# neofytr/LLMTokenizer

Measured on AMD Instinct MI355X. Metric: corpus MB/s per merge iter (train), 1 GiB synthetic corpus, higher is better.
Workload: dtype u32

## Files before the change

### llmtokenizer_amd/csrc/batch.hip

```cpp
#pragma once
#include "engine_common.h"

namespace bpeamd {

static_assert(TOPK == 64, "a wave holds a list, one entry per lane");
static_assert(BRB == 2 * (1024 / 64), "the select's 16 waves merge two partial lists each");
#ifndef BPE_SU
#define BPE_SU 1
#endif
#ifndef BPE_FORM_PRINT
#define BPE_FORM_PRINT 0
#endif
#ifndef BPE_RU
#define BPE_RU 4
#endif
#ifndef BPE_AU
#define BPE_AU 1
#endif
constexpr uint32_t AU = BPE_AU;
constexpr uint32_t SU = BPE_SU;
#ifndef BPE_RUN_THREAD_PAIRS
#define BPE_RUN_THREAD_PAIRS 16
#endif
constexpr uint32_t RUN_THREAD_PAIRS = BPE_RUN_THREAD_PAIRS, RUN_Q = 256;
// ... 691 lines not shown
        const unsigned long long pcut = sh && ovm < k ? bank_shfl(pre, ovm - 1) : 0ull;
        unsigned long long sumlen = 0;
#pragma unroll
        for (uint32_t b = 0; b < NBK; b++) {
            const uint32_t q = 64 * b + lane;
            slot_k[b] = slot[b];
            if (sh && q >= ovm) len[b] = slot_k[b] = 0;
            if (sh && ovm < k && q >= ovm) pre[b] = pcut;
            sumlen += q < k ? len[b] : 0u;
        }
        const unsigned long long stage_end = bank_shfl(pre, k - 1);
        sumlen = wave_sum(sumlen);
        uint32_t wk[NBK];
        unsigned long long sumw = 0, big = 0;
#pragma unroll
        for (uint32_t b = 0; b < NBK; b++) {
            const uint32_t q = 64 * b + lane;
            wk[b] = q < k && mode[b] != 0 && E->scan_occd ? min(len[b], fm_c[q] + len[b] / E->scan_occd) : len[b];
            sumw += q < k ? wk[b] : 0u;
        }
        sumw = wave_sum(sumw);
#pragma unroll
        for (uint32_t b = 0; b < NBK; b++) {
            const uint32_t q = 64 * b + lane;
            nb[b] = q < k ? 1 + (uint32_t)(sumw ? (uint64_t)(BSB - k) * wk[b] / sumw : 0) : 0;
            bpre[b] = nb[b];
            if (q < k) big = max(big, ((unsigned long long)wk[b] << 8) | (255u - q));
        }
        bank_scan(bpre);
        for (int o = 32; o > 0; o >>= 1) big = max(big, (unsigned long long)__shfl_xor(big, o));
        const uint32_t used = bank_shfl(bpre, k - 1);
        const uint32_t bigm = 255u - (uint32_t)(big & 255u);
        const uint32_t extra = BSB - used;
#pragma unroll
        for (uint32_t b = 0; b < NBK; b++) {
            const uint32_t q = 64 * b + lane;
            if (q < k) {
                B->a[q] = fm_u[q];
                B->b[q] = fm_v[q];
                B->cnt[q] = fm_c[q];
                B->mode[q] = mode[b];
                B->off[q] = off[b];
                B->len[q] = len[b];
                B->sbase[q] = (uint32_t)(pre[b] - slot_k[b]);
                B->R[q] = 0;
                B->bound[q] = 0;
                B->blk0[q] = bpre[b] - nb[b] + (q > bigm ? extra : 0);
                B->tmask[q] = (uint8_t)fm_tm[q];
                B->tspan[q] = (uint32_t)min(fm_span[q], 0xFFFFFFFFull);
                ctl[q] = tl[b];
            }
        }
        const uint32_t nsk = k ? fm_nsk[k - 1] : 0u;
        if (lane == 0) {
            B->sbase[k] = (uint32_t)stage_end;
            B->blk0[k] = BSB;
            B->sumlen = (uint32_t)sumlen;
            B->over = ovm < k ? ovm : BK;
            B->tpend = tpend < k ? tpend : BK;
            Bg->nsk = nsk;
            Bg->gr_n = 0;
#pragma unroll
            for (uint32_t g = 0; g < GRUN; g++) {
                Bg->gr_tk[g] = 0;
                Bg->gr_endc[g] = 0xFFFFFFFFu;
                Bg->gr_ready[g] = 0;
            }
            B->ztot = 0;
            B->tbar = 0;
            B->tlog_n = 0;
            B->why[why_end]++;
            if (ties > 1) C->counters[2]++;
        }
        ts_mark(E, bi, BT_SEL_CAND, false);
    }
    if (tid < 64 && stop != STOP_NONE) k = 0;
    if (tid == 0) {
        if (B->sc_out && B->ap_out) {
            B->sc_ticks += B->sc_out - ~B->sc_in;
            B->ap_ticks += B->ap_out - ~B->ap_in;
            B->nspan++;
        }
        B->sc_in = B->sc_out = B->ap_in = B->ap_out = 0;
        B->rhold = stop != STOP_NONE ? retry : 0u;
        Bg->nstall = nst;
        if (stalled && !C->err) C->err = 10;
        B->skgate = (stop == STOP_NONE && !retry && skg ? skg - 1u : skg) | (ske << 16);
        if (applied) {
            B->zrate = (uint32_t)min(2ull * B->nzero / (md ? md : 1u) + 2ull, 1ull << 20);
            Bg->crate = (uint32_t)min((unsigned long long)E->crate_pct * Bg->ncre / (100ull * (md ? md : 1u)) + 16ull, 1ull << 20);
            C->merges_done = md;
            C->occ_top += (uint32_t)rs;
            C->n_live = n_live;
            C->D = D;
            C->counters[0] += jst;
            C->counters[4] += oldsum;
            C->relist_c0 += rescan + ocand;
            C->relist_o0 += oocc;
            C->counters[5] += rs;
            if (jst) {
                C->a = olda;
                C->b = oldb;
                C->z = oldz0 + jst - 1;
            }
            if (retry) {
                B->nretry++;
                B->ndrop += kpr - retry;
            } else {
                B->nbatch++;
                B->ndrop += kpr - jst;
                Bg->nskip += oldnsk;
            }
            B->retry = 0;
            B->applied = 0;
            B->dD = 0;
        }
// ... 316 lines not shown

template <bool SH>
__device__ inline uint32_t cover_of(const uint32_t *__restrict__ tok, const RoleTab &rt, const BHalo &H, uint32_t p,
                                    int64_t ps, int64_t n) {
    if (!(rt.get(p) >> 31)) return BK;
    const int64_t pps = v_left<SH>(tok, ps);
    const uint32_t pp = tok_at_b<SH>(tok, H, pps, n);
    const uint32_t mm = rt.member(pp, p);
    if (mm >= BK || pp != p) return mm;
    uint32_t L;
    if (SH && ps < 0) {
        L = H.hlr[mm];
    } else {
        L = 1;
        int64_t x = v_left<SH>(tok, ps);
        for (; x >= 0 && tok[x] == p; x = v_left<SH>(tok, x)) L++;
        if (SH && x < 0) L += H.hlr[mm];
    }
    return (L & 1) ? BK : mm;
}

template <bool SH>
__device__ inline uint32_t starts_of(const uint32_t *__restrict__ tok, const RoleTab &rt, const BHalo &H, uint32_t q,
                                     int64_t kq, int64_t n) {
    const uint32_t lq = rt.get(q) & 0x7FFFFFFFu;
    if (!lq) return BK;
    const int64_t kn = v_right(kq, lq, n);
    return rt.member(q, tok_at_b<SH>(tok, H, kn, n));
}

enum : uint32_t { GRF_LGO = 1, GRF_LEND = 2, GRF_IGO = 3, GRF_IEND = 4 };
__device__ void bscan_long_runs(const Eng *__restrict__ E, Bat *__restrict__ B, const uint32_t *__restrict__ tok,
                                const RoleTab &rt, const BHalo &H, int64_t n, uint32_t z0, uint32_t sgen) {
    const uint32_t lane = threadIdx.x & 63;
    const uint32_t ng = uni(min(aload(&B->gr_n), GRUN));
    const uint64_t stride = gr_stride(E->n0), maxch = stride - 1;
    auto flag_of = [&](uint32_t st) { return (sgen << 3) | st; };
    for (uint32_t gi = 0; gi < ng; gi++) {
        uint32_t ok = 1;
        if (lane == 0) {
            const unsigned long long t0 = wall_clock64();
            while (__hip_atomic_load(&B->gr_ready[gi], __ATOMIC_ACQUIRE, __HIP_MEMORY_SCOPE_AGENT) != sgen) {
                if (wall_clock64() - t0 > E->gr_wait) {
                    ok = 0;
                    B->ra_err = 11;
                    atomicAdd(&B->gr_tready, 1u);
                    break;
                }
                __builtin_amdgcn_s_sleep(1);
            }
        }
        if (!uni((uint32_t)__shfl((int)ok, 0))) return;
        const uint32_t mg = uni(aload(&B->gr_m[gi])), ag = uni(B->a[mg]), zg = z0 + mg;
        const int64_t c0 = uni(aload(&B->gr_c[gi])), lag = uni(E->tlen[ag]);
        uint32_t *occg = E->ids_out + B->sbase[mg];
        uint16_t *tagg = E->btag + B->sbase[mg];
        const uint32_t slice = B->sbase[mg + 1] - B->sbase[mg];
        uint32_t *flags = E->grflag + (uint64_t)gi * stride;
        auto pos = [&](int64_t l) -> int64_t { return c0 + l * lag; };
        auto tk = [&](int64_t l) -> uint32_t {
            const int64_t p = pos(l);
            return p < n ? tok[p] : HOLE;
        };
        for (;;) {
            uint32_t chl = 0, endl = 0;
            if (lane == 0) {
                chl = atomicAdd(&B->gr_tk[gi], 1u);
// ... 101 lines not shown
                    npairs++;
                    if (q != HOLE) {
                        if (q == ag) nint_dr++;
                        else vadd_g(E, mg, V_DR, q, 1u);
                        if (rq == zg) nint_ir++;
                        else vadd_g(E, mg, V_IR, rq, 1u);
                    }
                }
              }
            }
            nint_dr = wave_sum(nint_dr);
            nint_ir = wave_sum(nint_ir);
            npairs = wave_sum(npairs);
            if (lane == 0) {
                vadd_g(E, mg, V_DR, ag, nint_dr);
                vadd_g(E, mg, V_IR, zg, nint_ir);
                if (npairs) atomicAdd(&B->bound[mg], npairs);
                atomicAdd(&B->nchunks, 1ull);
            }
#pragma unroll
            for (uint32_t bb = 0; bb < NBK; bb++) {
                unsigned long long tm = tadj.w[bb];
                for (int o = 32; o > 0; o >>= 1) tm |= __shfl_xor(tm, o);
                if (lane == 0 && tm) atomicOr(&B->adj[mg][bb], tm);
            }
        }
    }
}

template <bool SH>
__global__ __launch_bounds__(SCAN_T) void k_bscan(const Eng *__restrict__ E, const Ctl *__restrict__ C) {
    if (C->stop) return;
    Bat *B = E->bat;
    const uint32_t bi = bat_idx(E);
    ts_mark(E, bi, BT_SCAN_IN, true);
    if (threadIdx.x == 0) atomicMax(&B->sc_in, ~wall_clock64());
    __shared__ uint32_t s[4][DENSE];
    __shared__ uint32_t list[SCAN_T * SU * FR];
    __shared__ uint16_t ltag[SCAN_T * SU * FR];
    __shared__ uint32_t lcount, gbase, list_n, covc, sm, sk, sz0, bRs;
    __shared__ uint32_t lr_n, lr_brk, lr_pos[RUN_Q];
    __shared__ unsigned long long badj[NBK];
    __shared__ uint32_t gcnt[2];
    __shared__ uint32_t sa[BK], sb[BK];
    __shared__ RoleTab rt;
    __shared__ BHalo H;
    __shared__ uint32_t wmx[2][16];
    const uint32_t tid = threadIdx.x;
    const uint32_t sgen = ((uint32_t)(B->nbatch + B->nretry) & 0x0FFFFFFFu) + 1u;
    if (tid == 0) {
        sm = BK;
        covc = lcount = bRs = 0;
        lr_n = 0;
#pragma unroll
        for (uint32_t b = 0; b < NBK; b++) badj[b] = 0;
        gcnt[0] = gcnt[1] = 0;
        sk = B->k;
        sz0 = B->z0;
    }
    for (uint32_t q = tid; q < RH; q += SCAN_T) {
        rt.id[q] = HOLE;
        rt.fl[q] = 0;
    }
    for (uint32_t q = tid; q < RP; q += SCAN_T) rt.pk[q] = 0;
    uint32_t mla = 0;
    if (tid < BK) {
        const uint32_t lo = B->blk0[tid], hi = B->blk0[tid + 1];
        const uint32_t ma = B->a[tid];
        sa[tid] = ma;
        sb[tid] = B->b[tid];
        mla = E->tlen[ma];
        if (blockIdx.x >= lo && blockIdx.x < hi && tid < B->k) sm = tid;
    }
    __syncthreads();
    const uint32_t k = sk, m = sm, z0 = sz0;
    if (m >= k) {
        if (tid == 0) atomicMax(&B->sc_out, wall_clock64());
        return;
    }
    MK tadj = mk_zero();
    if (tid < k) {
        rt.put(sa[tid], sb[tid], mla, tid);
        if (SH) {
            Halo h;
            shard_halo(E->erec, E->nshards, E->shard, sa[tid], &h);
            H.hlr[tid] = h.hlrun;
            H.myi[tid] = h.myidx;
            if (tid == 0)
                for (int q = 0; q < 3; q++) {
                    H.HL[q] = h.HL[q];
                    H.HR[q] = h.HR[q];
                }
        }
    }
    const uint32_t a = sa[m], b = sb[m], z = z0 + m;
    const uint32_t la = E->tlen[a], lb = E->tlen[b];
    const uint32_t mode = B->mode[m], off = B->off[m], len = B->len[m];
    const uint32_t bid = blockIdx.x - B->blk0[m], nblk = B->blk0[m + 1] - B->blk0[m];
    const uint32_t sbase = B->sbase[m];
    uint32_t *occz = E->ids_out + sbase;
    uint16_t *tagz = E->btag + sbase;
    const uint32_t sslice = B->sbase[m + 1] - sbase;
#define STG(IDX, WHERE) if ((IDX) >= sslice) { B->ra_err = 12; } else
    uint32_t *Rm = &B->R[m];
    const int64_t n = (int64_t)E->n0;
    const uint32_t *__restrict__ tok = E->tok;
    const uint32_t want = mode == 2 ? a : b;
    const uint32_t lim = min(DENSE, z0 + k);
    for (uint32_t v = 0; v < 4; v++)
        for (uint32_t x = tid; x < lim; x += SCAN_T) s[v][x] = 0;
    __syncthreads();
    auto tok_at = [&](int64_t p) -> uint32_t { return tok_at_b<SH>(tok, H, p, n); };

    if (a != b) {
        static_assert(SU == 1 && BPE_WFLUSH, "the wave-driven candidate loop: one entry per lane per round");
        const uint32_t stride = nblk * SCAN_T;
        const uint32_t lane = tid & 63, wbase = (tid >> 6) * 64 * FR;
        uint32_t wcnt = 0, wocc = 0;
        uint32_t nent[SU];
        uint16_t ntg[SU];
        uint32_t eS = bid * SCAN_T + (tid & ~63u);
        auto load1 = [&](uint32_t s0, uint32_t &en, uint16_t &tg) {
            const uint32_t e = s0 + lane;
            en = 0;
            tg = 0xFFFFu;
            if (e < len) {
                en = mode == 0 ? E->plist[off + e] : E->occ[off + e];
                if (mode) tg = E->occnb[off + e];
            }
        };
        uint32_t pent = 0;
        uint16_t ptg = 0xFFFFu;
        auto advance = [&]() {
            eS += stride;
            if (SCAN_PD > 1) {
                nent[0] = pent;
                ntg[0] = ptg;
                if (eS + stride < len) load1(eS + stride, pent, ptg);
            } else if (eS < len) {
                load1(eS, nent[0], ntg[0]);
            }
        };
        auto flush = [&]() {
            __builtin_amdgcn_fence(__ATOMIC_RELEASE, "wavefront");
            __builtin_amdgcn_wave_barrier();
            uint32_t g = 0;
            if (lane == 0 && wcnt) g = atomicAdd(Rm, wcnt);
            g = __shfl(g, 0);
            for (uint32_t q = lane; q < wcnt; q += 64) {
                STG(g + q, "wflush") {
                occz[g + q] = list[wbase + q];
                tagz[g + q] = ltag[wbase + q];
                }
            }
// ... 281 lines not shown
                    }
                }
            }
            return fb < U;
        };
        if (nlr > RUN_BLOCK_Q) {
            for (uint32_t qi = wv; qi < nlr; qi += SCAN_T / 64) {
                int64_t c = lr_pos[qi];
                while (!segs(c, 0, std::integral_constant<uint32_t, 1>{}, [](uint32_t) { return 1u; }))
                    c += 64 * (int64_t)la;
            }
        } else {
            constexpr uint32_t NS = SCAN_T / 64 * RUN_BU;
            for (uint32_t qi = 0; qi < nlr; qi++) {
                int64_t c = lr_pos[qi];
                for (;;) {
                    if (tid == 0) lr_brk = NS;
                    __syncthreads();
                    segs(c, 64 * RUN_BU * wv, std::integral_constant<uint32_t, RUN_BU>{}, [&](uint32_t fb) {
                        if (lane == 0 && fb < RUN_BU) atomicMin(&lr_brk, wv * RUN_BU + fb);
                        __syncthreads();
                        const uint32_t gb = lr_brk, w0 = wv * RUN_BU;
                        return gb < w0 ? 0u : min(RUN_BU, gb - w0 + 1);
                    });
                    const bool done = lr_brk < NS;
                    __syncthreads();
                    if (done) break;
                    c += (int64_t)NS * 64 * la;
                }
            }
        }
    }
    __syncthreads();
    if (!SH && E->grflag) bscan_long_runs(E, B, tok, rt, H, n, z0, sgen);
    ts_mark(E, bi, BT_SCAN_CAND, false, true);
    if (tid < SKMAX && tid < B->nsk && ((B->sk_cm[tid][m >> 6] >> (m & 63)) & 1ull)) {
        const uint32_t xs = B->sk_a[tid], ys = B->sk_b[tid];
        uint32_t d = 0;
        if (xs == b && ys < lim) d += s[V_DR][ys];
        if (ys == a && xs < lim) d += s[V_DL][xs];
        if (d) atomicAdd(SH ? &E->xbat[BK + tid] : &B->sdec[tid], d);
    }
    const uint32_t Wx = xbat_vw(z0 + k);
    uint32_t *xm = SH ? E->xbat + XBH + (uint64_t)m * xbat_member_words(Wx) : nullptr;
    if (SH && blockIdx.x == 0 && tid == 0) {
        uint32_t xlm = BK;
        const int64_t F1 = C->F1, L1 = C->L1;
        const uint32_t over = B->over;
        if (F1 < n) {
            const uint32_t tf = tok[F1], tl1 = tok[L1];
            for (uint32_t mm = 0; mm < k; mm++)
                if (H.HL[0] == sa[mm] && tf == sb[mm] && (sa[mm] != sb[mm] || (H.hlr[mm] & 1))) {
                    xlm = mm;
                    break;
                }
            for (uint32_t mm = 0; mm < k && mm < over; mm++) {
                if (!(tl1 == sa[mm] && H.HR[0] == sb[mm] && (sa[mm] != sb[mm] || !(H.myi[mm] & 1)))) continue;
                uint32_t *xo = E->xbat + XBH + (uint64_t)mm * xbat_member_words(Wx);
                const uint32_t zz = z0 + mm;
                const int64_t ps = v_left<SH>(tok, L1);
                const uint32_t p = tok_at(ps);
                uint32_t lfin = p, bnd = 1;
                if (p != HOLE) {
                    const uint32_t cv = cover_of<SH>(tok, rt, H, p, ps, n);
                    if (cv < BK) {
                        lfin = z0 + cv;
                        bnd = 2;
                    } else {
                        xadd(E, xo, Wx, mm, V_DL, p);
                        xadd(E, xo, Wx, mm, V_IL, p);
                    }
                }
                const uint32_t q = H.HR[1];
                uint32_t rfin = q;
                if (q != HOLE) {
                    const uint32_t st = starts_of<SH>(tok, rt, H, q, n + 1, n);
                    if (st < BK) rfin = z0 + st;
                    xadd(E, xo, Wx, mm, V_DR, q);
                    xadd(E, xo, Wx, mm, V_IR, rfin);
                }
                (void)zz;
                const uint32_t g = atomicAdd(&B->R[mm], 1u);
                E->ids_out[B->sbase[mm] + g] = (uint32_t)L1;
                E->btag[B->sbase[mm] + g] = nb_tag(lfin, rfin);
                atomicAdd(&xo[0], 1u);
                atomicAdd(&xo[1], bnd);
                break;
            }
        }
        B->xl_m = xlm;
        if (over < k) atomicAdd(&E->xbat[over], 1u);
    }
    if (k > 1) {
#pragma unroll
        for (uint32_t bb = 0; bb < NBK; bb++) {
            unsigned long long t = tadj.w[bb];
            for (int o = 32; o > 0; o >>= 1) t |= __shfl_xor(t, o);
            if ((tid & 63) == 0 && t) atomicOr(&badj[bb], t);
        }
        __syncthreads();
        if (tid < NBK && badj[tid]) atomicOr(&B->adj[m][tid], badj[tid]);
    }
    uint32_t *rep = SH ? xm + 2 : E->bvecd + (uint64_t)(m * BREPL + bid % BREPL) * 4 * DENSE;
    const uint32_t vstride = SH ? Wx : DENSE;
    uint32_t mxl = 0, mxr = 0;
    for (uint32_t v = 0; v < 4; v++)
        for (uint32_t x = tid; x < lim; x += SCAN_T) {
            const uint32_t c = s[v][x];
            if (c) atomicAdd(&rep[v * vstride + x], c);
            if (v == V_DL) mxl = max(mxl, c);
            if (v == V_DR) mxr = max(mxr, c);
        }
    if (SH && tid == 0 && bRs) atomicAdd(&xm[0], bRs);
    if (k > 1) {
        for (int o = 32; o > 0; o >>= 1) {
            mxl = max(mxl, (uint32_t)__shfl_xor(mxl, o));
            mxr = max(mxr, (uint32_t)__shfl_xor(mxr, o));
        }
        if ((tid & 63) == 0) {
            wmx[0][tid >> 6] = mxl;
            wmx[1][tid >> 6] = mxr;
        }
        __syncthreads();
        if (tid == 0) {
            uint32_t l = 0, r = 0;
            for (uint32_t q = 0; q < SCAN_T / 64; q++) {
                l = max(l, wmx[0][q]);
                r = max(r, wmx[1][q]);
            }
            atomicAdd(SH ? &xm[1] : &B->bound[m], max(l + gcnt[V_DL] + covc, r + gcnt[V_DR]));
        }
    }
    ts_mark(E, bi, BT_SCAN_OUT, false, true);
    asm volatile("s_waitcnt vmcnt(0)" ::: "memory");
    __syncthreads();
    if (tid == 0) atomicMax(&B->sc_out, wall_clock64());
}
template __global__ void k_bscan<false>(const Eng *, const Ctl *);
template __global__ void k_bscan<true>(const Eng *, const Ctl *);

constexpr uint32_t XSP_SHIFT = 23;
static_assert(4 * BK < (1u << (32 - XSP_SHIFT)), "member-vector index fits above the id");
__global__ __launch_bounds__(256) void k_bpack(const Eng *__restrict__ E, const Ctl *__restrict__ C) {
    if (C->stop) return;
    const Bat *B = E->bat;
    __shared__ uint32_t pre[BK * 4 + 1];
    __shared__ uint32_t written;
    const uint32_t k = B->k, tid = threadIdx.x, nmv = 4 * k;
    if (tid < 64) {
        constexpr uint32_t LP = 4 * NBK;
        uint32_t c[LP], sum = 0;
#pragma unroll
        for (uint32_t j = 0; j < LP; j++) {
            c[j] = LP * tid + j < nmv ? E->bvnl[LP * tid + j] : 0u;
            sum += c[j];
        }
        uint32_t incl = sum;
        for (int o = 1; o < 64; o <<= 1) {
            const uint32_t y = __shfl_up(incl, o);
            if ((int)tid >= o) incl += y;
        }
        uint32_t r = incl - sum;
#pragma unroll
        for (uint32_t j = 0; j < LP; j++) {
            if (LP * tid + j <= nmv) pre[LP * tid + j] = r;
            r += c[j];
        }
    }
    __syncthreads();
// ... 637 lines not shown
```

### llmtokenizer_amd/csrc/engine.hip

```cpp
#include <hip/hip_runtime.h>
#include <fcntl.h>
#include <unistd.h>
#include <cerrno>

#include <algorithm>
#include <chrono>
#include <cstdio>
#include <cstdlib>
#include <cstring>
#include <string>
#include <thread>
#include <vector>
#include <unordered_map>

#include <rocprim/rocprim.hpp>

#include "../../include/bpe_gpu.h"
#include "kernels.hip"
#include "batch.hip"
#include "encode.hip"
#include "encode_win.hip"
#include "encode_docs.hip"
#include "split.hip"

// ... 189 lines not shown
            }
            return isnew == 1;
        };
        if (newt && is_new()) atomicAdd(&newt[t], 1u);
        const uint32_t bt = (uint32_t)(murmur_pair(u, v) & (C->Bfin[t] - 1));
        const uint32_t fc = E->sfirst[s];
        for (uint32_t q = 0; q < nq; q++) {
            if (qs[q].t != t) continue;
            if ((qs[q].flags & 1) && fc < qs[q].firstc) atomicAdd(&rho[q], 1u);
            if ((qs[q].flags & 2) && bt < qs[q].bucket && is_new()) atomicAdd(&nbl[q], 1u);
            if ((qs[q].flags & 4) && bt == qs[q].bucket) {
                const uint32_t p = atomicAdd(nmates, 1u);
                if (p < mcap) mates[p] = Mate{q, u, v, fc, is_new() ? 1u : 0u, 0};
            }
        }
    }
}

}

struct bpe_gpu_ctx {
    int dev = 0;
    hipStream_t st = nullptr;
    bool own_stream = true;
    uint32_t fast = 0;
    bool mlog_on = false;
    uint32_t sharded = 0, shard = 0, nshards = 1;
    uint64_t ntot = 0;
    uint32_t xfused = 0;
    uint32_t sbatch = 0;
    uint64_t stage_cap = 0;
    const P2P *xp2p = nullptr;
    unsigned long long xtimeout = 0;
    Eng h{};
    Eng *dE = nullptr;
    Ctl *dC = nullptr;
    Ctl *hC = nullptr;
    volatile uint32_t *hprobe = nullptr;
    hipEvent_t ev_probe[2] = {};
    uint64_t n0 = 0;
    bool loaded = false;
    bool ids_ready = false;
    uint64_t ids_len = 0;
    bool docs_ready = false;
    uint64_t docs_n = 0;
    uint64_t *d_idoff = nullptr;
    uint64_t docs_info[8] = {};
    bool split_ready = false;
    uint64_t split_n = 0;
    uint64_t *d_split = nullptr;
    size_t split_cap = 0;
    size_t merges_done = 0;
    std::vector<std::pair<void *, size_t>> train_allocs;
    std::vector<std::pair<void *, size_t>> pool;
    bool zdefer = false;
    std::vector<std::pair<void *, size_t>> zpend;
    uint32_t *d_tileoff = nullptr;
    uint32_t *d_enc_pairs = nullptr;
    hipGraphExec_t g_plain = nullptr, g_tracked = nullptr, g_encode = nullptr, g_batch = nullptr;
    bool hot_fallback = false;
    uint32_t relists = 0;
    std::vector<uint64_t> events;
    std::vector<hipGraphExec_t> retired;
    bpe_gpu_stats stats{};
    bool profile = false;
    hipEvent_t ev[2][ITERS_PER_GRAPH][2] = {};
// ... 243 lines not shown
                    (c->sharded ? c->sbatch != 0 : h.spec_on && (c->fast || n0 >= TRACK_LIMIT || HOT_TRACKED))
                ? 1
                : 0;
    h.relist_stale = 0;
    const bool will_batch = getenv_int("BPE_BATCH", 1) && h.hot;
    const int relist_env = getenv_int("BPE_RELIST", will_batch ? 1 : 0);
    if (!encode && !c->sharded && n0 >= (1ull << 24) && relist_env) {
        const char *t = getenv("BPE_RELIST_STALE");
        const uint64_t dflt = will_batch ? std::max<uint64_t>(n0 / 10, 1) : (32u << 20);
        h.relist_stale = (uint32_t)std::min<uint64_t>(t ? (uint64_t)std::max(1L, atol(t)) : dflt, 0xFFFFFFFFull);
    }
    h.hot_parts = SPEC_RB;
    h.hot_target = HOT_TARGET;
    if (const char *t = getenv("BPE_HOT_TARGET")) h.hot_target = std::max(1, std::min(atoi(t), (int)HOT_TARGET));
    h.hot_slot = h.hot_hist = h.hotp_tie = nullptr;
    h.hotp_best = h.hotp_key = h.hotp_v2 = h.hotp_k2 = nullptr;
    if (h.hot) {
        if ((r = dalloc(c, &h.hot_slot, HOT_CAP, false))) return r;
        if ((r = dalloc(c, &h.hot_hist, HOT_BINS))) return r;
        if ((r = dalloc(c, &h.hotp_best, SPEC_RB))) return r;
        if ((r = dalloc(c, &h.hotp_key, SPEC_RB))) return r;
        if ((r = dalloc(c, &h.hotp_v2, SPEC_RB))) return r;
        if ((r = dalloc(c, &h.hotp_k2, SPEC_RB))) return r;
        if ((r = dalloc(c, &h.hotp_tie, SPEC_RB))) return r;
    }
    h.batch = getenv_int("BPE_BATCH", 1) && h.hot && h.vcap <= BATCH_VCAP_MAX && (!c->sharded || c->sbatch) &&
                      (c->sharded || c->fast || n0 >= TRACK_LIMIT)
                  ? 1
                  : 0;
    h.skip_on = (uint32_t)(getenv_int("BPE_SKIP", 1) != 0);
    if (h.skip_on && getenv_int("BPE_SKIP_TEST", 0)) h.skip_on = 2;
    h.skg_exp = (uint32_t)getenv_int("BPE_SKGATE", 2);
    h.scan_occd = (uint32_t)std::max(0, getenv_int("BPE_SCAN_OCCD", 6));
    h.scan_compact = (uint32_t)(getenv_int("BPE_SCAN_COMPACT", 1) != 0);
    {
        int nl = BK > 63 ? 2 : 1;
        if (getenv_int("BPE_LIST2", 0)) nl = std::max(nl, 2);
        nl = getenv_int("BPE_NLIST", nl);
        h.nlists = (uint32_t)std::max(1, std::min(nl, (int)NLIST));
    }
    h.tie_up = (uint32_t)(getenv_int("BPE_TIE_UP", 0) != 0);
    h.crate_pct = (uint32_t)std::max(100, getenv_int("BPE_CRATE_PCT", 200));
    h.lose_retry = (uint32_t)(getenv_int("BPE_TEST_LOSE_RETRY", 0) != 0);
    h.xbat = nullptr;
    h.xsp_out = h.xsp_in = nullptr;
    h.xsp_cap = 0;
    h.xsp_stride = 0;
    h.bat = nullptr;
    h.btag = nullptr;
    h.bvecd = h.bvec = h.bvlist = h.bvnl = nullptr;
    h.tlog = nullptr;
    h.grflag = nullptr;
    h.tlog_cap = 0;
    h.bvs = h.vcap > DENSE ? h.vcap - DENSE : 1;
    uint32_t bat_dt = 0, bat_split = 0;
    if (h.batch) {
        if ((r = dalloc(c, &h.bat, 1))) return r;
        if ((r = dalloc(c, &h.btag, n0, false))) return r;
        if ((r = dalloc(c, &h.bvecd, (size_t)BK * BREPL * 4 * DENSE))) return r;
        if ((r = dalloc(c, &h.bvec, (size_t)BK * 4 * h.bvs))) return r;
        if ((r = dalloc(c, &h.bvlist, (size_t)BK * 4 * h.bvs, false))) return r;
        if ((r = dalloc(c, &h.bvnl, (size_t)BK * 4))) return r;
        if (!c->sharded && getenv_int("BPE_GR", 1) && (r = dalloc(c, &h.grflag, (size_t)GRUN * gr_stride(n0)))) return r;
        {
            int khz = 0;
            (void)hipDeviceGetAttribute(&khz, hipDeviceAttributeWallClockRate, c->dev);
// ... 723 lines not shown
            if (c->h.hot && !HOT_TRACKED) {
                c->h.hot = 0;
                c->h.batch = 0;
                C.full = 1;
                if ((r = push_desc(c))) return r;
            } else if (c->h.batch) {
                c->h.batch = 0;
                if ((r = push_desc(c))) return r;
            }
            if ((r = push_ctl(c))) return r;
            launch_stats(c);
            launch_argmax_inputs(c);
            k_select<<<1, 1024, 0, c->st>>>(c->dE, c->dC, fused_graph(c, true) ? SEL_PLAIN : SEL_TRACKED);
            HIPCHK(hipGetLastError());
            need_scan = true;
            break;
        case STOP_GROW: {
            C.stop = STOP_NONE;
            note_event(c, BPE_GPU_EV_TABLE_GROW, C.merges_done);
            note_event(c, BPE_GPU_EV_HOT_REBUILD, C.merges_done);
            C.full = 1;
            if ((r = push_ctl(c))) return r;
            if ((r = grow_table(c, c->h.hcap * 4))) return r;
            if ((r = hot_rebuild(c))) return r;
            if ((r = select_next(c, !c->h.fast && C.n_live < TRACK_LIMIT && !fused_graph(c, true)))) return r;
            need_scan = !c->h.batch;
            break;
        }
        case STOP_RELIST:
            C.stop = STOP_NONE;
            note_event(c, BPE_GPU_EV_RELIST, C.merges_done);
            C.relist_c0 = (uint32_t)C.counters[4];
            C.relist_o0 = (uint32_t)C.counters[5];
            if ((r = push_ctl(c))) return r;
            if ((r = relist(c))) return r;
            if ((r = select_next(c, false))) return r;
            need_scan = !c->h.batch;
            break;
        case STOP_HOT:
            C.stop = STOP_NONE;
            note_event(c, BPE_GPU_EV_HOT_REBUILD, C.merges_done);
            if ((r = push_ctl(c))) return r;
            if ((r = hot_rebuild(c))) return r;
            if ((r = select_next(c, false))) return r;
            need_scan = !c->h.batch;
            break;
        case STOP_STATS:
            C.stop = STOP_NONE;
            if (c->h.lcap && C.lgen >= 0xFFFEu) {
                HIPCHK(hipMemsetAsync(c->h.lkey, 0, c->h.lcap * 8, c->st));
                HIPCHK(hipMemsetAsync(c->h.lfirst, 0xFF, c->h.lcap * 8, c->st));
                C.lgen = 0;
            }
            if ((r = push_ctl(c))) return r;
            launch_stats(c);
            k_select<<<1, 1024, 0, c->st>>>(c->dE, c->dC, fused_graph(c, true) ? SEL_PLAIN : SEL_TRACKED);
            HIPCHK(hipGetLastError());
            need_scan = true;
            break;
        case STOP_EVENT: {
            if (!C.stat_exact) {
                C.stop = STOP_NONE;
                if ((r = push_ctl(c))) return r;
                launch_stats(c);
                HIPCHK(hipGetLastError());
                if ((r = pull_ctl(c))) return r;
// ... 97 lines not shown
    c->stats.tie_failed = hb.ntfail;
    c->stats.keys_zeroed = hb.nzero;
    {
        unsigned long long t[2] = {0, 0};
        HIPCHK(hipMemcpy(t, &c->h.bat->nskip, 16, hipMemcpyDeviceToHost));
        c->stats.keys_skipped = t[0];
        c->stats.skip_failed = t[1];
    }
    {
        unsigned long long t[2] = {0, 0};
        HIPCHK(hipMemcpy(t, &c->h.bat->sl_ticks, 16, hipMemcpyDeviceToHost));
        int khz = 0;
        (void)hipDeviceGetAttribute(&khz, hipDeviceAttributeWallClockRate, c->dev);
        c->stats.select_launches = t[1];
        if (khz > 0 && t[1]) c->stats.ms_select_span = (double)t[0] / t[1] / khz;
    }
    if (hb.nspan) {
        int khz = 0;
        (void)hipDeviceGetAttribute(&khz, hipDeviceAttributeWallClockRate, c->dev);
        if (khz > 0) {
            c->stats.ms_scan_span = (double)hb.sc_ticks / hb.nspan / khz;
            c->stats.ms_apply_span = (double)hb.ap_ticks / hb.nspan / khz;
        }
    }
    if (c->h.dbgts) print_batch_timeline(c, hb.nbatch + hb.nretry);
    if (getenv("BPE_DEBUG") && c->h.grflag) {
        uint32_t g[4] = {0, 0, 0, 0};
        unsigned long long nch = 0;
        HIPCHK(hipMemcpy(g, &c->h.bat->gr_tready, 16, hipMemcpyDeviceToHost));
        HIPCHK(hipMemcpy(&nch, &c->h.bat->nchunks, 8, hipMemcpyDeviceToHost));
        fprintf(stderr, "long runs: %u registered, %llu chunks walked, wait timeouts %u (registration) %u (chunk)\n", g[2],
                nch, g[0], g[1]);
    }
    if (getenv("BPE_DEBUG"))
        fprintf(stderr, "batches %llu, dropped %llu, re-formed %llu; formation ended by: list %llu, cap/count/hot_T %llu, a==b %llu, "
                "duplicate %llu, tie %llu, conflict %llu, table margin %llu, staging %llu; tie-verified %llu (re-formed %llu); "
                "keys zeroed %llu; keys skipped %llu (re-formed %llu)\n", hb.nbatch, hb.ndrop, hb.nretry,
                hb.why[0], hb.why[1], hb.why[2], hb.why[3], hb.why[4], hb.why[5], hb.why[6], hb.why[7], hb.ntie, hb.ntfail,
                hb.nzero, (unsigned long long)c->stats.keys_skipped, (unsigned long long)c->stats.skip_failed);
    return 0;
}

void batch_profile(bpe_gpu_ctx *c) {
    if (!c->stats.batches) return;
    const double nl = (double)(c->stats.batches + c->stats.batch_retries);
    c->prof_name = "k_bscan";
    c->prof_ms = c->stats.ms_scan_span;
    c->prof_bytes = (8.0 * c->stats.candidates + 20.0 * c->stats.occurrences) / nl;
    c->prof_launches = (uint64_t)nl;
}

int compact_ids(bpe_gpu_ctx *c) {
    int r;
    const uint64_t ntl = c->h.ntiles;
    unsigned long long *d_status;
    if ((r = dalloc(c, &d_status, ntl + 1, false))) return r;
    uint32_t *d_ticket = reinterpret_cast<uint32_t *>(d_status + ntl);
    HIPCHK(hipMemsetAsync(d_status, 0, (ntl + 1) * 8, c->st));
    if (ntl) k_live_compact<<<(uint32_t)ntl, LC_T, 0, c->st>>>(c->dE, d_status, d_ticket, d_ticket + 1);
    HIPCHK(hipGetLastError());
    uint32_t tot = 0;
    HIPCHK(hipMemcpyAsync(&tot, d_ticket + 1, 4, hipMemcpyDeviceToHost, c->st));
    HIPCHK(hipStreamSynchronize(c->st));
    c->ids_len = tot;
    c->ids_ready = true;
    return 0;
// ... 1640 lines not shown
```

### llmtokenizer_amd/csrc/engine_common.h

```cpp
#pragma once
#include <hip/hip_runtime.h>
#include <stddef.h>
#include <stdint.h>

namespace bpeamd {

constexpr uint32_t HOLE = 0xFFFFFFFFu;
constexpr uint32_t END_FLAG = 0x80000000u;
constexpr uint32_t MARKV = 0xFFFFFFFEu;
constexpr uint64_t END_MAX = 0x7FFFFFFDull;
__host__ __device__ inline bool is_id(uint32_t v) { return v < END_FLAG; }
__host__ __device__ inline uint32_t end_code(uint64_t d) { return END_FLAG | (uint32_t)d; }
#ifndef BPE_DENSE
#define BPE_DENSE 8192
#endif
constexpr uint32_t DENSE = BPE_DENSE;
#ifndef BPE_REPL
#define BPE_REPL 8
#endif
constexpr uint32_t REPL = BPE_REPL;
constexpr uint32_t NTHR = 16;
constexpr uint64_t CHUNK = 65536;
constexpr uint64_t DYN_LIMIT = CHUNK * NTHR;
constexpr uint64_t TRACK_LIMIT = 2 * DYN_LIMIT;
// ... 42 lines not shown
    return (128u + m) << (e - 7);
}

enum : uint32_t { SEL_PLAIN = 0, SEL_TRACKED = 1, SEL_FUSED = 2 };

constexpr uint32_t BMAX = 512;
constexpr uint32_t BIDS = 2048;
constexpr uint32_t BPAIRS = 1024;

struct EncBatch {
    uint32_t nb, total, occ_base, r0;
    uint32_t nbg;
    uint32_t a[BMAX], b[BMAX], z[BMAX], mode[BMAX], off[BMAX], len[BMAX], la[BMAX], lb[BMAX];
    uint32_t seg[BMAX + 1];
    uint32_t R[BMAX];
};


constexpr uint32_t TOPK = 64;
#ifndef BPE_BK
#define BPE_BK 127
#endif
constexpr uint32_t BK = BPE_BK;
constexpr uint32_t NBK = (BK + 1) / 64;
static_assert(BK + 1 == 64 * NBK && NBK >= 1 && NBK <= 2, "BK is 63 or 127");
constexpr uint32_t SKMAX = BK;
#ifndef BPE_NLIST
#define BPE_NLIST 4
#endif
constexpr uint32_t NLIST = BPE_NLIST;
constexpr uint32_t BRB = 32;
constexpr uint32_t BREPL = 2;
constexpr uint32_t BSB = 256;
constexpr uint32_t STALL_LIMIT = 64;
constexpr uint32_t GRUN = 4;
constexpr uint32_t GR_CH = 16384;
constexpr uint32_t GR_PROBE = 4096;
__host__ __device__ inline uint64_t gr_stride(uint64_t n0) { return n0 / GR_CH + 2; }
constexpr uint32_t P2P_MAXR_B = 16;

struct Bat {
    uint32_t k, z0, applied, jstar;
    uint32_t ticket, retry, sumlen, rhold;
    unsigned long long dD;
    unsigned long long nbatch, ndrop, nretry;
    unsigned long long why[8];
    uint32_t drop_test;
    uint32_t skgate;
    unsigned long long stage_cap;
    unsigned long long sc_in, sc_out, ap_in, ap_out, sc_ticks, ap_ticks, nspan, nupd;
    uint32_t a[BK], b[BK], cnt[BK], mode[BK], off[BK], len[BK];
    uint32_t blk0[BK + 1];
    uint32_t sbase[BK + 1];
    uint32_t R[BK];
    uint32_t bound[BK];
    uint32_t Rg[BK];
    uint32_t over;
    uint32_t xl_m;
    uint32_t tpend;
    uint32_t ztot;
    uint32_t tbar, zrate;
    unsigned long long ntie, ntfail, nzero;
    uint8_t tmask[BK + 1];
    uint32_t tspan[BK];
    uint32_t tlog_n;
    unsigned long long pv[BRB * TOPK], pk[BRB * TOPK];
    uint32_t ra_k, ra_top, ra_done, ra_err;
    uint32_t ra_z[BK], ra_la[BK], ra_lb[BK], ra_R[BK], ra_sbase[BK], ra_pre[BK + 1];
    uint32_t ra_xl, ra_xlb;
    uint32_t ra_lo[BK];
    uint32_t ra_split;
    uint32_t nstall;
    unsigned long long sl_in, sl_out, sl_ticks, nsl;
    unsigned long long adj[BK][NBK];
    uint32_t mla[BK], mlb[BK];
    uint32_t nsk, skpad;
    uint32_t sk_a[SKMAX], sk_b[SKMAX], sk_c[SKMAX];
    uint32_t sdec[SKMAX];
    unsigned long long sk_cm[SKMAX][NBK];
    uint8_t nskb[BK + 1];
    unsigned long long nskip, nskfail;
    uint32_t cnew[BK];
    uint32_t crate;
// ... 56 lines not shown
    unsigned long long *dbgts;
    uint32_t dbg_form;
    uint32_t prefix_apply;
    uint32_t rw_hold;
    uint32_t rw_hold_max;
    uint32_t *tlog;
    uint32_t tlog_cap;
    uint32_t tie_verify;
    uint32_t *hprobe;
    uint32_t fast;
    uint32_t spec_on;
    uint32_t scan_blocks;
    uint32_t sharded, shard, nshards;
    uint32_t *xbuf;
    uint32_t xstride;
    uint32_t xfused;
    unsigned long long xtimeout;
    uint32_t *myrec;
    uint32_t *erec;
    const uint32_t *enc_pairs;
    uint32_t n_enc;
    EncBatch *eb;
    uint32_t hot;
    uint32_t hot_parts;
    uint32_t hot_target;
    uint32_t relist_stale;
    uint32_t *hot_slot;
    uint32_t *hot_hist;
    unsigned long long *hotp_best, *hotp_key, *hotp_v2, *hotp_k2;
    uint32_t *hotp_tie;
    uint32_t batch;
    uint32_t skip_on;
    uint32_t scan_compact;
    uint32_t scan_occd;
    uint32_t skg_exp;
    uint32_t nlists;
    uint32_t tie_up;
    uint32_t crate_pct;
    uint32_t lose_retry;
    uint32_t bvs;
    Bat *bat;
    uint16_t *btag;
    uint32_t *bvecd;
    uint32_t *bvec;
    uint32_t *bvlist;
    uint32_t *bvnl;
    uint32_t *xbat;
    uint32_t *grflag;
    unsigned long long gr_wait;
    uint32_t *xsp_out, *xsp_in;
    uint32_t xsp_cap, xsp_stride;
    uint64_t end_max;
    uint32_t track_ub;
    unsigned long long light_wait;
    unsigned long long *lkey, *lfirst;
    uint64_t lcap;
    unsigned long long *mlog;
    uint64_t mlog_cap;
};
constexpr uint32_t MLOG_WORDS = 5;
constexpr uint64_t MLOG_MAX = 1ull << 20;

struct Ctl {
    uint32_t a, b, z, stop;
    uint32_t merges_done, parity, R, occ_top;
    uint32_t cand_mode, cand_off, cand_len, stop_z;
// ... 185 lines not shown
```

Measured before the change: 119.9 million.

## Split scan work across blocks by weighted prefix so blocks cover several merges

```diff
diff --git a/llmtokenizer_amd/csrc/batch.hip b/llmtokenizer_amd/csrc/batch.hip
--- a/llmtokenizer_amd/csrc/batch.hip
+++ b/llmtokenizer_amd/csrc/batch.hip
@@ -747,10 +747,60 @@
         const uint32_t used = bank_shfl(bpre, k - 1);
         const uint32_t bigm = 255u - (uint32_t)(big & 255u);
         const uint32_t extra = BSB - used;
+        static_assert(SPLIT_CAP == 4, "the cap argument above: (SPLIT_CAP - 1) f >= T");
+        unsigned long long wpre[NBK];
+        unsigned long long splitT = 0;
+        uint32_t splitB0 = 0;
+        {
+            uint32_t apre[NBK];
+            unsigned long long w0 = 0;
+#pragma unroll
+            for (uint32_t b = 0; b < NBK; b++) {
+                const uint32_t q = 64 * b + lane;
+                const bool aa = q < k && fm_u[q] == fm_v[q];
+                apre[b] = aa ? nb[b] : 0u;
+                w0 += q < k && !aa && len[b] ? wk[b] : 0u;
+            }
+            bank_scan(apre);
+            w0 = wave_sum(w0);
+            const uint32_t Ba = k ? bank_shfl(apre, k - 1) : 0u, Bf = BSB - Ba;
+            const unsigned long long den = 3ull * Bf > k ? 3ull * Bf - k : 0ull;
+            const unsigned long long f = den ? (w0 + Bf + den - 1) / den : 0ull;
+#pragma unroll
+            for (uint32_t b = 0; b < NBK; b++) {
+                const uint32_t q = 64 * b + lane;
+                const bool aa = q < k && fm_u[q] == fm_v[q];
+                wpre[b] = q < k && !aa && len[b] ? max((unsigned long long)wk[b], f) : 0ull;
+            }
+            bank_scan(wpre);
+            const unsigned long long W = k ? bank_shfl(wpre, k - 1) : 0ull;
+            const unsigned long long T = Bf ? (W + Bf - 1) / Bf : 0ull;
+            bool slow = false;
+#pragma unroll
+            for (uint32_t b = 0; b < NBK; b++) {
+                const uint32_t q = 64 * b + lane;
+                const bool aa = q < k && fm_u[q] == fm_v[q];
+                const unsigned long long nbq = nb[b] + (q == bigm ? extra : 0u);
+                slow = slow || (q < k && !aa && len[b] && 100ull * wk[b] > E->scan_split_pct * T * nbq);
+            }
+            const bool pays = E->scan_split >= 2 || __ballot(slow) != 0ull;
+            if (E->scan_split && pays && k && den && w0 && T && 3ull * f >= T) {
+                splitT = T;
+                splitB0 = Ba;
+#pragma unroll
+                for (uint32_t b = 0; b < NBK; b++) {
+                    const uint32_t q = 64 * b + lane;
+                    const bool aa = q < k && fm_u[q] == fm_v[q];
+                    bpre[b] = apre[b];
+                    if (!aa) nb[b] = 0;
+                }
+            }
+        }
 #pragma unroll
         for (uint32_t b = 0; b < NBK; b++) {
             const uint32_t q = 64 * b + lane;
             if (q < k) {
+                B->wpre[q + 1] = wpre[b];
                 B->a[q] = fm_u[q];
                 B->b[q] = fm_v[q];
                 B->cnt[q] = fm_c[q];
@@ -760,7 +810,7 @@
                 B->sbase[q] = (uint32_t)(pre[b] - slot_k[b]);
                 B->R[q] = 0;
                 B->bound[q] = 0;
-                B->blk0[q] = bpre[b] - nb[b] + (q > bigm ? extra : 0);
+                B->blk0[q] = bpre[b] - nb[b] + (!splitT && q > bigm ? extra : 0);
                 B->tmask[q] = (uint8_t)fm_tm[q];
                 B->tspan[q] = (uint32_t)min(fm_span[q], 0xFFFFFFFFull);
                 ctl[q] = tl[b];
@@ -769,7 +819,11 @@
         const uint32_t nsk = k ? fm_nsk[k - 1] : 0u;
         if (lane == 0) {
             B->sbase[k] = (uint32_t)stage_end;
-            B->blk0[k] = BSB;
+            B->blk0[k] = splitT ? splitB0 : BSB;
+            B->wpre[0] = 0;
+            B->split_T = splitT;
+            if (splitT) B->nsplit++;
+            B->split_b0 = splitB0;
             B->sumlen = (uint32_t)sumlen;
             B->over = ovm < k ? ovm : BK;
             B->tpend = tpend < k ? tpend : BK;
@@ -793,10 +847,11 @@
     if (tid == 0) {
         if (B->sc_out && B->ap_out) {
             B->sc_ticks += B->sc_out - ~B->sc_in;
+            B->sc_btk += B->sc_blk;
             B->ap_ticks += B->ap_out - ~B->ap_in;
             B->nspan++;
         }
-        B->sc_in = B->sc_out = B->ap_in = B->ap_out = 0;
+        B->sc_in = B->sc_out = B->ap_in = B->ap_out = B->sc_blk = 0;
         B->rhold = stop != STOP_NONE ? retry : 0u;
         Bg->nstall = nst;
         if (stalled && !C->err) C->err = 10;
@@ -1179,7 +1234,8 @@
 enum : uint32_t { GRF_LGO = 1, GRF_LEND = 2, GRF_IGO = 3, GRF_IEND = 4 };
 __device__ void bscan_long_runs(const Eng *__restrict__ E, Bat *__restrict__ B, const uint32_t *__restrict__ tok,
                                 const RoleTab &rt, const BHalo &H, int64_t n, uint32_t z0, uint32_t sgen) {
-    const uint32_t lane = threadIdx.x & 63;
+    uint32_t lane = threadIdx.x & 63;
+    asm volatile("" : "+v"(lane));
     const uint32_t ng = uni(min(aload(&B->gr_n), GRUN));
     const uint64_t stride = gr_stride(E->n0), maxch = stride - 1;
     auto flag_of = [&](uint32_t st) { return (sgen << 3) | st; };
@@ -1347,13 +1403,17 @@
 __global__ __launch_bounds__(SCAN_T) void k_bscan(const Eng *__restrict__ E, const Ctl *__restrict__ C) {
     if (C->stop) return;
     Bat *B = E->bat;
-    const uint32_t bi = bat_idx(E);
+    const uint32_t bi = uni(bat_idx(E));
     ts_mark(E, bi, BT_SCAN_IN, true);
-    if (threadIdx.x == 0) atomicMax(&B->sc_in, ~wall_clock64());
+    if (threadIdx.x == 0) {
+        const unsigned long long t_in = wall_clock64();
+        atomicMax(&B->sc_in, ~t_in);
+        atomicAdd(&B->sc_blk, 0ull - t_in);
+    }
     __shared__ uint32_t s[4][DENSE];
     __shared__ uint32_t list[SCAN_T * SU * FR];
     __shared__ uint16_t ltag[SCAN_T * SU * FR];
-    __shared__ uint32_t lcount, gbase, list_n, covc, sm, sk, sz0, bRs;
+    __shared__ uint32_t lcount, gbase, list_n, covc, sk, sz0, bRs;
     __shared__ uint32_t lr_n, lr_brk, lr_pos[RUN_Q];
     __shared__ unsigned long long badj[NBK];
     __shared__ uint32_t gcnt[2];
@@ -1361,15 +1421,11 @@
     __shared__ RoleTab rt;
     __shared__ BHalo H;
     __shared__ uint32_t wmx[2][16];
+    __shared__ uint32_t pc_n, pc_m[SPLIT_CAP], pc_u0[SPLIT_CAP], pc_us[SPLIT_CAP], pc_ue[SPLIT_CAP], pc_rep[SPLIT_CAP];
     const uint32_t tid = threadIdx.x;
-    const uint32_t sgen = ((uint32_t)(B->nbatch + B->nretry) & 0x0FFFFFFFu) + 1u;
+    const uint32_t sgen = uni(((uint32_t)(B->nbatch + B->nretry) & 0x0FFFFFFFu) + 1u);
     if (tid == 0) {
-        sm = BK;
-        covc = lcount = bRs = 0;
-        lr_n = 0;
-#pragma unroll
-        for (uint32_t b = 0; b < NBK; b++) badj[b] = 0;
-        gcnt[0] = gcnt[1] = 0;
+        pc_n = 0;
         sk = B->k;
         sz0 = B->z0;
     }
@@ -1380,20 +1436,59 @@
     for (uint32_t q = tid; q < RP; q += SCAN_T) rt.pk[q] = 0;
     uint32_t mla = 0;
     if (tid < BK) {
-        const uint32_t lo = B->blk0[tid], hi = B->blk0[tid + 1];
         const uint32_t ma = B->a[tid];
         sa[tid] = ma;
         sb[tid] = B->b[tid];
         mla = E->tlen[ma];
-        if (blockIdx.x >= lo && blockIdx.x < hi && tid < B->k) sm = tid;
     }
     __syncthreads();
-    const uint32_t k = sk, m = sm, z0 = sz0;
-    if (m >= k) {
-        if (tid == 0) atomicMax(&B->sc_out, wall_clock64());
+    if (tid < sk) {
+        const uint32_t lo = B->blk0[tid], hi = B->blk0[tid + 1];
+        const uint32_t U = (B->len[tid] + SCAN_UNIT - 1) / SCAN_UNIT;
+        const unsigned long long T = B->split_T;
+        uint32_t u0 = 0, us = 0, ue = 0, rep = 0;
+        if (blockIdx.x >= lo && blockIdx.x < hi) {
+            u0 = (blockIdx.x - lo) * (SCAN_T / SCAN_UNIT);
+            us = (hi - lo) * (SCAN_T / SCAN_UNIT);
+            ue = max(U, 1u);
+            rep = (blockIdx.x - lo) % BREPL;
+        } else if (T && blockIdx.x >= B->split_b0 && sa[tid] != sb[tid]) {
+            const unsigned long long P = B->wpre[tid], w = B->wpre[tid + 1] - P;
+            const unsigned long long r0 = (unsigned long long)(blockIdx.x - B->split_b0) * T, r1 = r0 + T;
+            if (w && r0 < P + w && r1 > P) {
+                const unsigned long long x0 = r0 > P ? r0 - P : 0ull, x1 = min(r1 - P, w);
+                u0 = (uint32_t)((x0 * U + w - 1) / w);
+                ue = (uint32_t)((x1 * U + w - 1) / w);
+                us = SCAN_T / SCAN_UNIT;
+                rep = blockIdx.x % BREPL;
+            }
+        }
+        if (u0 < ue) {
+            const uint32_t pi = atomicAdd(&pc_n, 1u);
+            if (pi < SPLIT_CAP) {
+                pc_m[pi] = tid;
+                pc_u0[pi] = u0;
+                pc_us[pi] = us;
+                pc_ue[pi] = ue;
+                pc_rep[pi] = rep;
+            } else {
+                B->ra_err = 12;
+            }
+        }
+    }
+    __syncthreads();
+    const uint32_t k = uni(sk), z0 = uni(sz0), npc = uni(min(pc_n, SPLIT_CAP));
+    auto stamp_out = [&]() {
+        if (tid == 0) {
+            const unsigned long long t_out = wall_clock64();
+            atomicMax(&B->sc_out, t_out);
+            atomicAdd(&B->sc_blk, t_out);
+        }
+    };
+    if (npc == 0 && !(SH && blockIdx.x == 0 && k > 0)) {
+        stamp_out();
         return;
     }
-    MK tadj = mk_zero();
     if (tid < k) {
         rt.put(sa[tid], sb[tid], mla, tid);
         if (SH) {
@@ -1408,33 +1503,48 @@
                 }
         }
     }
-    const uint32_t a = sa[m], b = sb[m], z = z0 + m;
-    const uint32_t la = E->tlen[a], lb = E->tlen[b];
-    const uint32_t mode = B->mode[m], off = B->off[m], len = B->len[m];
-    const uint32_t bid = blockIdx.x - B->blk0[m], nblk = B->blk0[m + 1] - B->blk0[m];
-    const uint32_t sbase = B->sbase[m];
+    const int64_t n = (int64_t)E->n0;
+    const uint32_t *__restrict__ tok = E->tok;
+    const uint32_t lim = uni(min(DENSE, z0 + k));
+    const uint32_t Wx = uni(xbat_vw(z0 + k));
+    auto tok_at = [&](int64_t p) -> uint32_t { return tok_at_b<SH>(tok, H, p, n); };
+    for (uint32_t pi = 0; pi < npc; pi++) {
+    __syncthreads();
+    const uint32_t m = uni(pc_m[pi]);
+    if (tid == 0) {
+        covc = lcount = bRs = 0;
+        lr_n = 0;
+        unsigned long long z64 = 0;
+        asm volatile("" : "+v"(z64));
+#pragma unroll
+        for (uint32_t bb = 0; bb < NBK; bb++) badj[bb] = z64;
+        gcnt[0] = gcnt[1] = 0;
+    }
+    MK tadj = mk_zero();
+    const uint32_t a = uni(sa[m]), b = uni(sb[m]), z = z0 + m;
+    const uint32_t la = uni(E->tlen[a]), lb = uni(E->tlen[b]);
+    const uint32_t mode = uni(B->mode[m]), off = uni(B->off[m]);
+    const uint32_t len = uni((uint32_t)min((uint64_t)B->len[m], (uint64_t)pc_ue[pi] * SCAN_UNIT));
+    const uint32_t bid = uni(pc_u0[pi] / (SCAN_T / SCAN_UNIT)), nblk = uni(pc_us[pi] / (SCAN_T / SCAN_UNIT));
+    const uint32_t sbase = uni(B->sbase[m]);
     uint32_t *occz = E->ids_out + sbase;
     uint16_t *tagz = E->btag + sbase;
-    const uint32_t sslice = B->sbase[m + 1] - sbase;
+    const uint32_t sslice = uni(B->sbase[m + 1]) - sbase;
 #define STG(IDX, WHERE) if ((IDX) >= sslice) { B->ra_err = 12; } else
     uint32_t *Rm = &B->R[m];
-    const int64_t n = (int64_t)E->n0;
-    const uint32_t *__restrict__ tok = E->tok;
     const uint32_t want = mode == 2 ? a : b;
-    const uint32_t lim = min(DENSE, z0 + k);
     for (uint32_t v = 0; v < 4; v++)
         for (uint32_t x = tid; x < lim; x += SCAN_T) s[v][x] = 0;
     __syncthreads();
-    auto tok_at = [&](int64_t p) -> uint32_t { return tok_at_b<SH>(tok, H, p, n); };
 
     if (a != b) {
         static_assert(SU == 1 && BPE_WFLUSH, "the wave-driven candidate loop: one entry per lane per round");
-        const uint32_t stride = nblk * SCAN_T;
+        const uint32_t stride = uni(pc_us[pi] * SCAN_UNIT);
         const uint32_t lane = tid & 63, wbase = (tid >> 6) * 64 * FR;
         uint32_t wcnt = 0, wocc = 0;
         uint32_t nent[SU];
         uint16_t ntg[SU];
-        uint32_t eS = bid * SCAN_T + (tid & ~63u);
+        uint32_t eS = pc_u0[pi] * SCAN_UNIT + (tid & ~63u);
         auto load1 = [&](uint32_t s0, uint32_t &en, uint16_t &tg) {
             const uint32_t e = s0 + lane;
             en = 0;
@@ -1782,17 +1892,59 @@
         }
     }
     __syncthreads();
-    if (!SH && E->grflag) bscan_long_runs(E, B, tok, rt, H, n, z0, sgen);
-    ts_mark(E, bi, BT_SCAN_CAND, false, true);
-    if (tid < SKMAX && tid < B->nsk && ((B->sk_cm[tid][m >> 6] >> (m & 63)) & 1ull)) {
-        const uint32_t xs = B->sk_a[tid], ys = B->sk_b[tid];
+    uint32_t et = tid;
+    asm volatile("" : "+v"(et));
+    if (et < SKMAX && et < B->nsk && ((B->sk_cm[et][m >> 6] >> (m & 63)) & 1ull)) {
+        const uint32_t xs = B->sk_a[et], ys = B->sk_b[et];
         uint32_t d = 0;
         if (xs == b && ys < lim) d += s[V_DR][ys];
         if (ys == a && xs < lim) d += s[V_DL][xs];
-        if (d) atomicAdd(SH ? &E->xbat[BK + tid] : &B->sdec[tid], d);
-    }
-    const uint32_t Wx = xbat_vw(z0 + k);
+        if (d) atomicAdd(SH ? &E->xbat[BK + et] : &B->sdec[et], d);
+    }
     uint32_t *xm = SH ? E->xbat + XBH + (uint64_t)m * xbat_member_words(Wx) : nullptr;
+    if (k > 1) {
+#pragma unroll
+        for (uint32_t bb = 0; bb < NBK; bb++) {
+            unsigned long long t = tadj.w[bb];
+            for (int o = 32; o > 0; o >>= 1) t |= __shfl_xor(t, o);
+            if ((et & 63) == 0 && t) atomicOr(&badj[bb], t);
+        }
+        __syncthreads();
+        if (et < NBK && badj[et]) atomicOr(&B->adj[m][et], badj[et]);
+    }
+    uint32_t *rep = SH ? xm + 2 : E->bvecd + (uint64_t)(m * BREPL + pc_rep[pi]) * 4 * DENSE;
+    const uint32_t vstride = SH ? Wx : DENSE;
+    uint32_t mxl = 0, mxr = 0;
+    for (uint32_t v = 0; v < 4; v++)
+        for (uint32_t x = et; x < lim; x += SCAN_T) {
+            const uint32_t c = s[v][x];
+            if (c) atomicAdd(&rep[v * vstride + x], c);
+            if (v == V_DL) mxl = max(mxl, c);
+            if (v == V_DR) mxr = max(mxr, c);
+        }
+    if (SH && et == 0 && bRs) atomicAdd(&xm[0], bRs);
+    if (k > 1) {
+        for (int o = 32; o > 0; o >>= 1) {
+            mxl = max(mxl, (uint32_t)__shfl_xor(mxl, o));
+            mxr = max(mxr, (uint32_t)__shfl_xor(mxr, o));
+        }
+        if ((et & 63) == 0) {
+            wmx[0][et >> 6] = mxl;
+            wmx[1][et >> 6] = mxr;
+        }
+        __syncthreads();
+        if (et == 0) {
+            uint32_t l = 0, r = 0;
+            for (uint32_t q = 0; q < SCAN_T / 64; q++) {
+                l = max(l, wmx[0][q]);
+                r = max(r, wmx[1][q]);
+            }
+            atomicAdd(SH ? &xm[1] : &B->bound[m], max(l + gcnt[V_DL] + covc, r + gcnt[V_DR]));
+        }
+    }
+    }
+#undef STG
+    __syncthreads();
     if (SH && blockIdx.x == 0 && tid == 0) {
         uint32_t xlm = BK;
         const int64_t F1 = C->F1, L1 = C->L1;
@@ -1841,50 +1993,12 @@
         B->xl_m = xlm;
         if (over < k) atomicAdd(&E->xbat[over], 1u);
     }
-    if (k > 1) {
-#pragma unroll
-        for (uint32_t bb = 0; bb < NBK; bb++) {
-            unsigned long long t = tadj.w[bb];
-            for (int o = 32; o > 0; o >>= 1) t |= __shfl_xor(t, o);
-            if ((tid & 63) == 0 && t) atomicOr(&badj[bb], t);
-        }
-        __syncthreads();
-        if (tid < NBK && badj[tid]) atomicOr(&B->adj[m][tid], badj[tid]);
-    }
-    uint32_t *rep = SH ? xm + 2 : E->bvecd + (uint64_t)(m * BREPL + bid % BREPL) * 4 * DENSE;
-    const uint32_t vstride = SH ? Wx : DENSE;
-    uint32_t mxl = 0, mxr = 0;
-    for (uint32_t v = 0; v < 4; v++)
-        for (uint32_t x = tid; x < lim; x += SCAN_T) {
-            const uint32_t c = s[v][x];
-            if (c) atomicAdd(&rep[v * vstride + x], c);
-            if (v == V_DL) mxl = max(mxl, c);
-            if (v == V_DR) mxr = max(mxr, c);
-        }
-    if (SH && tid == 0 && bRs) atomicAdd(&xm[0], bRs);
-    if (k > 1) {
-        for (int o = 32; o > 0; o >>= 1) {
-            mxl = max(mxl, (uint32_t)__shfl_xor(mxl, o));
-            mxr = max(mxr, (uint32_t)__shfl_xor(mxr, o));
-        }
-        if ((tid & 63) == 0) {
-            wmx[0][tid >> 6] = mxl;
-            wmx[1][tid >> 6] = mxr;
-        }
-        __syncthreads();
-        if (tid == 0) {
-            uint32_t l = 0, r = 0;
-            for (uint32_t q = 0; q < SCAN_T / 64; q++) {
-                l = max(l, wmx[0][q]);
-                r = max(r, wmx[1][q]);
-            }
-            atomicAdd(SH ? &xm[1] : &B->bound[m], max(l + gcnt[V_DL] + covc, r + gcnt[V_DR]));
-        }
-    }
+    if (!SH && E->grflag) bscan_long_runs(E, B, tok, rt, H, n, z0, sgen);
+    ts_mark(E, bi, BT_SCAN_CAND, false, true);
     ts_mark(E, bi, BT_SCAN_OUT, false, true);
     asm volatile("s_waitcnt vmcnt(0)" ::: "memory");
     __syncthreads();
-    if (tid == 0) atomicMax(&B->sc_out, wall_clock64());
+    stamp_out();
 }
 template __global__ void k_bscan<false>(const Eng *, const Ctl *);
 template __global__ void k_bscan<true>(const Eng *, const Ctl *);
diff --git a/llmtokenizer_amd/csrc/engine.hip b/llmtokenizer_amd/csrc/engine.hip
--- a/llmtokenizer_amd/csrc/engine.hip
+++ b/llmtokenizer_amd/csrc/engine.hip
@@ -245,6 +245,8 @@
     uint64_t stage_cap = 0;
     const P2P *xp2p = nullptr;
     unsigned long long xtimeout = 0;
+    unsigned long long dbg_relist_sc[2] = {0, 0};
+    bool dbg_relisted = false;
     Eng h{};
     Eng *dE = nullptr;
     Ctl *dC = nullptr;
@@ -554,6 +556,8 @@
     if (h.skip_on && getenv_int("BPE_SKIP_TEST", 0)) h.skip_on = 2;
     h.skg_exp = (uint32_t)getenv_int("BPE_SKGATE", 2);
     h.scan_occd = (uint32_t)std::max(0, getenv_int("BPE_SCAN_OCCD", 6));
+    h.scan_split = (uint32_t)std::min(2, std::max(0, getenv_int("BPE_SCAN_SPLIT", 1)));
+    h.scan_split_pct = (uint32_t)std::max(100, getenv_int("BPE_SCAN_SPLIT_PCT", 125));
     h.scan_compact = (uint32_t)(getenv_int("BPE_SCAN_COMPACT", 1) != 0);
     {
         int nl = BK > 63 ? 2 : 1;
@@ -1343,6 +1347,11 @@
             note_event(c, BPE_GPU_EV_RELIST, C.merges_done);
             C.relist_c0 = (uint32_t)C.counters[4];
             C.relist_o0 = (uint32_t)C.counters[5];
+            if (c->h.batch && !c->dbg_relisted && getenv("BPE_DEBUG")) {
+                HIPCHK(hipMemcpy(&c->dbg_relist_sc[0], &c->h.bat->sc_ticks, 8, hipMemcpyDeviceToHost));
+                HIPCHK(hipMemcpy(&c->dbg_relist_sc[1], &c->h.bat->sc_btk, 8, hipMemcpyDeviceToHost));
+                c->dbg_relisted = true;
+            }
             if ((r = push_ctl(c))) return r;
             if ((r = relist(c))) return r;
             if ((r = select_next(c, false))) return r;
@@ -1506,6 +1515,15 @@
         fprintf(stderr, "long runs: %u registered, %llu chunks walked, wait timeouts %u (registration) %u (chunk)\n", g[2],
                 nch, g[0], g[1]);
     }
+    if (getenv("BPE_DEBUG")) {
+        auto util = [](unsigned long long blk, unsigned long long span) { return span ? (double)blk / ((double)BSB * (double)span) : 0.0; };
+        const unsigned long long s0 = c->dbg_relisted ? c->dbg_relist_sc[0] : hb.sc_ticks;
+        const unsigned long long b0 = c->dbg_relisted ? c->dbg_relist_sc[1] : hb.sc_btk;
+        fprintf(stderr, "scan utilisation (split rule %u: %llu batches cut) = %.4f over %llu scans; before the list rebuild %.4f "
+                "(%.1f%% of the span ticks), after it %.4f\n", c->h.scan_split, hb.nsplit, util(hb.sc_btk, hb.sc_ticks), hb.nspan, util(b0, s0),
+                hb.sc_ticks ? 100.0 * (double)s0 / (double)hb.sc_ticks : 0.0, util(hb.sc_btk - b0, hb.sc_ticks - s0));
+    }
+    c->dbg_relisted = false;
     if (getenv("BPE_DEBUG"))
         fprintf(stderr, "batches %llu, dropped %llu, re-formed %llu; formation ended by: list %llu, cap/count/hot_T %llu, a==b %llu, "
                 "duplicate %llu, tie %llu, conflict %llu, table margin %llu, staging %llu; tie-verified %llu (re-formed %llu); "
diff --git a/llmtokenizer_amd/csrc/engine_common.h b/llmtokenizer_amd/csrc/engine_common.h
--- a/llmtokenizer_amd/csrc/engine_common.h
+++ b/llmtokenizer_amd/csrc/engine_common.h
@@ -98,6 +98,8 @@
 constexpr uint32_t BRB = 32;
 constexpr uint32_t BREPL = 2;
 constexpr uint32_t BSB = 256;
+constexpr uint32_t SCAN_UNIT = 64;
+constexpr uint32_t SPLIT_CAP = 4;
 constexpr uint32_t STALL_LIMIT = 64;
 constexpr uint32_t GRUN = 4;
 constexpr uint32_t GR_CH = 16384;
@@ -115,6 +117,10 @@
     uint32_t skgate;
     unsigned long long stage_cap;
     unsigned long long sc_in, sc_out, ap_in, ap_out, sc_ticks, ap_ticks, nspan, nupd;
+    unsigned long long sc_blk, sc_btk;
+    unsigned long long split_T, wpre[BK + 1];
+    uint32_t split_b0, split_pad;
+    unsigned long long nsplit;
     uint32_t a[BK], b[BK], cnt[BK], mode[BK], off[BK], len[BK];
     uint32_t blk0[BK + 1];
     uint32_t sbase[BK + 1];
@@ -237,6 +243,8 @@
     uint32_t batch;
     uint32_t skip_on;
     uint32_t scan_compact;
+    uint32_t scan_split;
+    uint32_t scan_split_pct;
     uint32_t scan_occd;
     uint32_t skg_exp;
     uint32_t nlists;
```

Measured after the change: 121.7 million (median of 6 runs). +1.4%, better.
